# Merium88/3D-Object-Detection-of-Industrial-Joints

Measured on NVIDIA B200. Metric: SHOT descriptors/s + scene registrations/s at 1-8 B200 vs PCL OMP host CPU, higher is better.
Workload: dtype f32 (f64 for the SHOT frame/bin decisions)

## Files before the change

### 3d-object-detection-of-industrial-joints_b200/csrc/shot.cu

```cuda
#include <algorithm>

#include "linalg3.cuh"
#include "search.cuh"

namespace {

constexpr int SHOT_THREADS = 128;
constexpr int SHOT_LEN = 352;

__global__ void gather_normals_kernel(const float4 *__restrict__ sorted_pts, int n, const float4 *__restrict__ normals,
                                      float4 *__restrict__ out) {
  int i = blockIdx.x * blockDim.x + threadIdx.x;
  if (i < n) out[i] = normals[orig_index(sorted_pts[i])];
}

struct FloatBins {
  float *h;
  __device__ __forceinline__ void add(int bin, float v) const { atomicAdd(&h[bin], v); }
};
struct FixedBins {
  int *h;
  float scale;
  __device__ __forceinline__ void add(int bin, float v) const { atomicAdd(&h[bin], __float2int_rn(v * scale)); }
};

template <class Bins>
__device__ __noinline__ void shot_neighbor_exact(Bins s_hist, const float4 nv, const float4 p, const float4 c,
                                                 const float d2, const float *fr, const double radius) {
  const float fxx = fr[0], fxy = fr[1], fxz = fr[2];
  const float fyx = fr[3], fyy = fr[4], fyz = fr[5];
  const float fzx = fr[6], fzy = fr[7], fzz = fr[8];
  const double radius3_4 = (radius * 3) / 4, radius1_4 = radius / 4, radius1_2 = radius / 2;
  const double RAD_45 = 0.78539816339744830961566084581988;
  const double RAD_90 = 1.5707963267948966192313216916398;
  const double RAD_135 = 2.3561944901923449288469825374596;
  const double RAD_PI_7_8 = 2.7488935718910690836548129603691;
  {
        float dotf = nv.x * fzx;
        dotf += nv.y * fzy;
        dotf += nv.z * fzz;
        double cosineDesc = (double)dotf;
        if (cosineDesc > 1.0) cosineDesc = 1.0;
        if (cosineDesc < -1.0) cosineDesc = -1.0;
        double binDistance = ((1.0 + cosineDesc) * 10) / 2;
        const float dx = p.x - c.x, dy = p.y - c.y, dz = p.z - c.z;
        const double distance = sqrt((double)d2);
        if (fabs(distance) < 1E-15) return;
        float t;
        t = dx * fxx;
        t += dy * fxy;
        t += dz * fxz;
        double xInFeatRef = (double)t;
        t = dx * fyx;
        t += dy * fyy;
        t += dz * fyz;
        double yInFeatRef = (double)t;
        t = dx * fzx;
        t += dy * fzy;
        t += dz * fzz;
        double zInFeatRef = (double)t;
        if (fabs(yInFeatRef) < 1E-30) yInFeatRef = 0;
        if (fabs(xInFeatRef) < 1E-30) xInFeatRef = 0;
        if (fabs(zInFeatRef) < 1E-30) zInFeatRef = 0;

        const int bit4 = ((yInFeatRef > 0) || ((yInFeatRef == 0.0) && (xInFeatRef < 0))) ? 1 : 0;
        const int bit3 = (((xInFeatRef > 0) || ((xInFeatRef == 0.0) && (yInFeatRef > 0))) ? !bit4 : bit4) ? 1 : 0;
        int desc_index = (bit4 << 3) + (bit3 << 2);
        desc_index = desc_index << 1;
        if ((xInFeatRef * yInFeatRef > 0) || (xInFeatRef == 0.0))
          desc_index += (fabs(xInFeatRef) >= fabs(yInFeatRef)) ? 0 : 4;
        else
          desc_index += (fabs(xInFeatRef) > fabs(yInFeatRef)) ? 4 : 0;
        desc_index += zInFeatRef > 0 ? 1 : 0;
        desc_index += (distance > radius1_2) ? 2 : 0;

        const int step_index = (int)floor(binDistance + 0.5);
        const int volume_index = desc_index * 11;
        binDistance -= step_index;
        double intWeight = (1 - fabs(binDistance));
        if (binDistance > 0)
          s_hist.add(volume_index + ((step_index + 1) % 10), (float)binDistance);
        else
          s_hist.add(volume_index + ((step_index - 1 + 10) % 10), -(float)binDistance);
// ... 163 lines not shown
        if (pz) atomicAdd(&s_votes[2], pz);
      }
      __syncthreads();
      if (tid == 0) {
        double ax[2][3] = {{v1x, v1y, v1z}, {v3x, v3y, v3z}};
        for (int which = 0; which < 2; ++which) {
          int plus = 2 * s_votes[1 + which] - valid;
          double *a = ax[which];
          if (plus == 0) {
            const int med = valid / 2;
            for (int t = -2; t <= 2; ++t) {
              const float4 p = pts[pos[n_skip + med - t]];
              const double vx = (double)(p.x - c.x), vy = (double)(p.y - c.y), vz = (double)(p.z - c.z);
              if (vx * a[0] + vy * a[1] + vz * a[2] > 0) ++plus;
            }
            if (plus < 3) {
              a[0] = -a[0];
              a[1] = -a[1];
              a[2] = -a[2];
            }
          } else if (plus < 0) {
            a[0] = -a[0];
            a[1] = -a[1];
            a[2] = -a[2];
          }
        }
        const float x0 = (float)ax[0][0], x1 = (float)ax[0][1], x2 = (float)ax[0][2];
        const float z0 = (float)ax[1][0], z1 = (float)ax[1][1], z2 = (float)ax[1][2];
        s_frame[0] = x0;
        s_frame[1] = x1;
        s_frame[2] = x2;
        s_frame[3] = z1 * x2 - z2 * x1;
        s_frame[4] = z2 * x0 - z0 * x2;
        s_frame[5] = z0 * x1 - z1 * x0;
        s_frame[6] = z0;
        s_frame[7] = z1;
        s_frame[8] = z2;
      }
      __syncthreads();
    }

    if (lrf_only) {
      if (tid < 9) rf_out[(size_t)i * 9 + tid] = ok ? s_frame[tid] : nanf32();
      __syncthreads();
      continue;
    }

    const bool desc_ok = ok && n >= 5;
    if (desc_ok) {
      float fr[9];
#pragma unroll
      for (int a = 0; a < 9; ++a) fr[a] = s_frame[a];
      for (int j = tid; j < n; j += SHOT_THREADS) {
        const int pj = pos[j];
        const float4 nv = nrm[pj];
        if (!finite3(nv.x, nv.y, nv.z)) continue;
        shot_neighbor_exact(FloatBins{s_hist}, nv, pts[pj], c, key_d2(key[j]), fr, radius);
      }
      __syncthreads();
      double acc = 0.0;
      for (int b = tid; b < SHOT_LEN; b += SHOT_THREADS) {
        const float h = s_hist[b];
        acc += (double)(h * h);
      }
      acc = warp_sum(acc);
      if ((tid & 31) == 0) s_norm[tid >> 5] = acc;
      __syncthreads();
      const double acc_norm = sqrt(((s_norm[0] + s_norm[1]) + s_norm[2]) + s_norm[3]);
      const float fnorm = (float)acc_norm;
      for (int b = tid; b < SHOT_LEN; b += SHOT_THREADS) desc[(size_t)i * SHOT_LEN + b] = s_hist[b] / fnorm;
      if (rf_out && tid < 9) rf_out[(size_t)i * 9 + tid] = s_frame[tid];
    } else {
      for (int b = tid; b < SHOT_LEN; b += SHOT_THREADS) desc[(size_t)i * SHOT_LEN + b] = nanf32();
      if (rf_out && tid < 9) rf_out[(size_t)i * 9 + tid] = nanf32();
    }
    __syncthreads();
  }
}

constexpr int SW_WARPS = 8;
constexpr int SW_THREADS = SW_WARPS * 32;
constexpr int SW_CAP = 2016;

__global__ void __launch_bounds__(256)
    shot_count_cov_kernel(GridView g, const float4 *__restrict__ kp, int K, float radius_f, double radius, float r2,
                          int *__restrict__ counts, double *__restrict__ acc, unsigned long long *__restrict__ stats) {
  const int i = (blockIdx.x * blockDim.x + threadIdx.x) >> 5;
  const int lane = threadIdx.x & 31;
  if (i >= K) return;
  const float4 c = kp[i];
  double part[7] = {0, 0, 0, 0, 0, 0, 0};
  int n = 0, skipped = 0;
  int x0, x1, y0, y1, z0, z1;
  if (finite3(c.x, c.y, c.z) && g.n > 0 && ball_cell_range(g, c.x, c.y, c.z, radius_f, x0, x1, y0, y1, z0, z1)) {
    const float4 *__restrict__ pts = g.pts;
    const int *__restrict__ cs = g.cell_start;
    for (int z = z0; z <= z1; ++z)
      for (int y = y0; y <= y1; ++y) {
        const int base = g.dx * (y + g.dy * z);
        const int e = cs[base + x1 + 1];
        for (int j0 = cs[base + x0] + lane; j0 < e; j0 += 128) {
         float4 pp[4];
#pragma unroll
         for (int u = 0; u < 4; ++u) pp[u] = (j0 + 32 * u < e) ? pts[j0 + 32 * u] : make_float4(0.f, 0.f, 0.f, 0.f);
#pragma unroll
         for (int u = 0; u < 4; ++u) {
          const float4 p = pp[u];
          const float d2 = (j0 + 32 * u < e) ? sqdist3(c.x, c.y, c.z, p.x, p.y, p.z) : 3.0e38f;
          if (d2 < r2) {
            ++n;
            if (p.x == c.x && p.y == c.y && p.z == c.z) {
              ++skipped;
            } else {
              const double vx = (double)(p.x - c.x), vy = (double)(p.y - c.y), vz = (double)(p.z - c.z);
              const double w = radius - sqrt((double)d2);
              part[0] += w * (vx * vx);
              part[1] += w * (vx * vy);
              part[2] += w * (vx * vz);
              part[3] += w * (vy * vy);
              part[4] += w * (vy * vz);
              part[5] += w * (vz * vz);
              part[6] += w;
            }
          }
         }
        }
      }
  }
#pragma unroll
  for (int a = 0; a < 7; ++a) part[a] = warp_sum(part[a]);
  n = warp_sum(n);
  skipped = warp_sum(skipped);
  if (lane < 7) {
    double v = part[0];
#pragma unroll
    for (int a = 1; a < 7; ++a)
      if (lane == a) v = part[a];
    acc[(size_t)i * 8 + lane] = v;
  }
  if (lane == 7) acc[(size_t)i * 8 + 7] = (double)skipped;
  if (lane == 0) {
    counts[i] = n;
    if (stats) {
      atomicMax(&stats[0], (unsigned long long)n);
      atomicAdd(&stats[1], (unsigned long long)n);
    }
  }
}

__global__ void shot_eigen_kernel(const int *__restrict__ counts, const double *__restrict__ acc, int K,
                                  double *__restrict__ axes, int *__restrict__ flags) {
  const int i = blockIdx.x * blockDim.x + threadIdx.x;
  if (i >= K) return;
  const double *s = acc + (size_t)i * 8;
  const int valid = counts[i] - (int)s[7];
  int ok = valid >= 5 ? 1 : 0;
  double ax[6] = {0, 0, 0, 0, 0, 0};
  if (ok) {
    const double cov[9] = {s[0] / s[6], s[1] / s[6], s[2] / s[6], s[1] / s[6], s[3] / s[6],
                           s[4] / s[6], s[2] / s[6], s[4] / s[6], s[5] / s[6]};
    double w[3], V[9];
    eigh3_f64(cov, w, V);
    if (!isfinite(w[0]) || !isfinite(w[1]) || !isfinite(w[2])) ok = 0;
    ax[0] = V[0 * 3 + 2], ax[1] = V[1 * 3 + 2], ax[2] = V[2 * 3 + 2];
    ax[3] = V[0 * 3 + 0], ax[4] = V[1 * 3 + 0], ax[5] = V[2 * 3 + 0];
  }
#pragma unroll
  for (int a = 0; a < 6; ++a) axes[(size_t)i * 6 + a] = ax[a];
  flags[i] = ok;
}

struct ShotWarpSmem {
  int pos[SW_CAP];
  int hist[SHOT_LEN];
  int sel[8];
};

__global__ void __launch_bounds__(SW_THREADS, 3)
    shot_warp_kernel(GridView g, const float4 *__restrict__ nrm, const float4 *__restrict__ kp,
                     const int *__restrict__ counts, const double *__restrict__ acc, const double *__restrict__ axes,
                     const int *__restrict__ flags, int K, float radius_f, double radius, float r2,
                     int *__restrict__ work_counter, float *__restrict__ desc, float *__restrict__ rf_out,
                     int lrf_only) {
  extern __shared__ __align__(16) unsigned char smem_raw[];
  const int lane = threadIdx.x & 31, warp = threadIdx.x >> 5;
  ShotWarpSmem &sm = reinterpret_cast<ShotWarpSmem *>(smem_raw)[warp];
  const float4 *__restrict__ pts = g.pts;
  const int *__restrict__ cs = g.cell_start;

  const double radius3_4 = (radius * 3) / 4, radius1_4 = radius / 4, radius1_2 = radius / 2;
  const float r12f = (float)radius1_2, r34f = (float)radius3_4, r14f = (float)radius1_4;
  const float inv_r12f = 1.0f / r12f;
  const float m_r = 1e-6f * radius_f;
  const float RAD_45f = 0.78539816339744830961566084581988f, RAD_90f = 1.5707963267948966192313216916398f;
  const float RAD_135f = 2.3561944901923449288469825374596f, RAD_PI_7_8f = 2.7488935718910690836548129603691f;
  const float INV_RAD_90f = 1.0f / RAD_90f, INV_RAD_45f = 1.0f / RAD_45f;
  const float COS_45f = 0.70710678118654752440f;

  while (true) {
    int i = 0;
    if (lane == 0) i = atomicAdd(work_counter, 1);
    i = __shfl_sync(0xffffffffu, i, 0);
    if (i >= K) break;
    if (counts[i] > SW_CAP) continue;
    const float4 c = kp[i];

    int n = 0;
    {
      int x0, x1, y0, y1, z0, z1;
      if (finite3(c.x, c.y, c.z) && g.n > 0 && ball_cell_range(g, c.x, c.y, c.z, radius_f, x0, x1, y0, y1, z0, z1)) {
        for (int z = z0; z <= z1; ++z)
          for (int y = y0; y <= y1; ++y) {
            const int base = g.dx * (y + g.dy * z);
            const int s0 = cs[base + x0], e = cs[base + x1 + 1];
            for (int j0 = s0; j0 < e; j0 += 128) {
              float4 p[4];
#pragma unroll
              for (int u = 0; u < 4; ++u) {
                const int j = j0 + 32 * u + lane;
                p[u] = (j < e) ? pts[j] : make_float4(0.f, 0.f, 0.f, 0.f);
              }
#pragma unroll
              for (int u = 0; u < 4; ++u) {
                const int j = j0 + 32 * u + lane;
                const bool hit = j < e && sqdist3(c.x, c.y, c.z, p[u].x, p[u].y, p[u].z) < r2;
                const unsigned m = __ballot_sync(0xffffffffu, hit);
                if (hit) {
                  const int slot = n + __popc(m & ((1u << lane) - 1u));
                  if (slot < SW_CAP) sm.pos[slot] = j;
                }
                n += __popc(m);
              }
            }
          }
      }
    }
    if (n > SW_CAP) n = SW_CAP;
    for (int b = lane; b < SHOT_LEN; b += 32) sm.hist[b] = 0;
    __syncwarp();

    const int n_skip = (int)acc[(size_t)i * 8 + 7];
    const int valid = n - n_skip;
    const int ok = flags[i];
    double ax[6];
#pragma unroll
    for (int a = 0; a < 6; ++a) ax[a] = axes[(size_t)i * 6 + a];
    float fr[9];
    if (ok) {
      const float a0 = (float)ax[0], a1 = (float)ax[1], a2 = (float)ax[2];
      const float b0 = (float)ax[3], b1 = (float)ax[4], b2 = (float)ax[5];
      int px = 0, pz = 0;
      for (int j = lane; j < n; j += 32) {
        const float4 p = pts[sm.pos[j]];
        if (p.x == c.x && p.y == c.y && p.z == c.z) continue;
        const float fx = p.x - c.x, fy = p.y - c.y, fz = p.z - c.z;
        const float band = 4e-6f * (fabsf(fx) + fabsf(fy) + fabsf(fz));
        const float ex = fx * a0 + fy * a1 + fz * a2, ez = fx * b0 + fy * b1 + fz * b2;
        if (fabsf(ex) > band)
          px += ex > 0.f;
        else
          px += ((double)fx * ax[0] + (double)fy * ax[1] + (double)fz * ax[2] >= 0) ? 1 : 0;
        if (fabsf(ez) > band)
          pz += ez > 0.f;
        else
          pz += ((double)fx * ax[3] + (double)fy * ax[4] + (double)fz * ax[5] >= 0) ? 1 : 0;
      }
      px = warp_sum(px);
      pz = warp_sum(pz);
      const int plus_x = 2 * px - valid, plus_z = 2 * pz - valid;
      if (plus_x == 0 || plus_z == 0) {
        const int r0 = n_skip + valid / 2 - 2;
        const bool staged = n <= SW_CAP / 2;
        float *d2s = reinterpret_cast<float *>(sm.pos + SW_CAP / 2);
        auto d2_at = [&](int a) -> float {
          if (staged) return d2s[a];
          const float4 q = pts[sm.pos[a]];
          return sqdist3(c.x, c.y, c.z, q.x, q.y, q.z);
        };
        if (staged) {
          for (int a = lane; a < n; a += 32) {
            const float4 q = pts[sm.pos[a]];
            d2s[a] = sqdist3(c.x, c.y, c.z, q.x, q.y, q.z);
          }
          __syncwarp();
        }
        unsigned u_lo = 0, u_hi = 0;
#pragma unroll 1
        for (int which = 0; which < 2; ++which) {
          const int target = r0 + 4 * which + 1;
          unsigned lo = 0, hi = 0x7f800000u;
          while (lo < hi) {
// ... 145 lines not shown
            hist.add((desc_index - 2) * 11 + step_index, -rd);
          }
        } else {
          const float rd = (df - r14f) * inv_r12f;
          if (df < r14f)
            intWeight += 1 + rd;
          else {
            intWeight += 1 - rd;
            hist.add((desc_index + 2) * 11 + step_index, rd);
          }
        }
        const float inc = acosf(fminf(1.0f, fmaxf(-1.0f, cosv)));
        if (zf < 0.f) {
          const float id = (inc - RAD_135f) * INV_RAD_90f;
          if (cosv < -COS_45f)
            intWeight += 1 - id;
          else {
            intWeight += 1 + id;
            hist.add((desc_index + 1) * 11 + step_index, -id);
          }
        } else {
          const float id = (inc - RAD_45f) * INV_RAD_90f;
          if (cosv > COS_45f)
            intWeight += 1 + id;
          else {
            intWeight += 1 - id;
            hist.add((desc_index - 1) * 11 + step_index, id);
          }
        }
        {
          float ad = (az - az0) * INV_RAD_45f;
          ad = fmaxf(-0.5f, fminf(ad, 0.5f));
          if (ad > 0) {
            intWeight += 1 - ad;
            hist.add(((desc_index + 4) % 32) * 11 + step_index, ad);
          } else {
            intWeight += 1 + ad;
            hist.add(((desc_index - 4 + 32) % 32) * 11 + step_index, -ad);
          }
        }
        hist.add(volume_index + step_index, intWeight);
      }
      __syncwarp();
      double acc = 0.0;
      for (int b = lane; b < SHOT_LEN; b += 32) {
        const float h = (float)(unsigned)sm.hist[b] * fx_inv;
        acc += (double)(h * h);
      }
      acc = warp_sum(acc);
      const float fnorm = (float)sqrt(acc);
      for (int b = lane; b < SHOT_LEN; b += 32)
        desc[(size_t)i * SHOT_LEN + b] = ((float)(unsigned)sm.hist[b] * fx_inv) / fnorm;
      if (rf_out && lane < 9) {
        float v = 0.f;
#pragma unroll
        for (int a = 0; a < 9; ++a)
          if (lane == a) v = fr[a];
        rf_out[(size_t)i * 9 + lane] = v;
      }
    } else {
      for (int b = lane; b < SHOT_LEN; b += 32) desc[(size_t)i * SHOT_LEN + b] = nanf32();
      if (rf_out && lane < 9) rf_out[(size_t)i * 9 + lane] = nanf32();
    }
    __syncwarp();
  }
}

}

int dev_shot(b200_ctx *ctx, b200_cloud *c, const float *d_normals, const float4 *d_kp, int K, double radius,
             float *d_desc, float *d_rf, bool lrf_only) {
  if (!(radius > 0.0)) return ctx->fail(B200_ERR_INVALID, "shot: radius must be > 0");
  if (K <= 0) return B200_OK;
  const GridView *g;
  B200_TRY(cloud_grid_for_radius(c, radius, &g));
  DevBuf<int> counts, flags;
  DevBuf<double> acc, axes;
  DevBuf<unsigned long long> stats;
  B200_TRY(counts.alloc(ctx, (size_t)K));
  B200_TRY(flags.alloc(ctx, (size_t)K));
  B200_TRY(acc.alloc(ctx, (size_t)K * 8));
  B200_TRY(axes.alloc(ctx, (size_t)K * 6));
  B200_TRY(stats.alloc(ctx, 2));
  const float r2 = (float)(radius * radius);
  {
    StageScope stc_(ctx, ST_NBR_COUNT);
    B200_CUDA(ctx, cudaMemsetAsync(stats.p, 0, 2 * sizeof(unsigned long long), ctx->stream));
    shot_count_cov_kernel<<<ceil_div((long long)K * 32, 256), 256, 0, ctx->stream>>>(*g, d_kp, K, (float)radius, radius,
                                                                                    r2, counts.p, acc.p, stats.p);
    B200_LAUNCHED(ctx);
    shot_eigen_kernel<<<ceil_div(K, 128), 128, 0, ctx->stream>>>(counts.p, acc.p, K, axes.p, flags.p);
    B200_LAUNCHED(ctx);
  }
  unsigned long long hstats[2];
  B200_TRY(readback_small(ctx, stats.p, hstats, sizeof(hstats)));
  const int max_count = (int)hstats[0];
  ctx->last_max_nbrs = max_count;
  ctx->last_mean_nbrs = (double)hstats[1] / K;

  StageScope st_(ctx, ST_SHOT);
  DevBuf<float4> nrm_sorted;
  if (!lrf_only) {
    B200_TRY(nrm_sorted.alloc(ctx, (size_t)std::max(c->n_valid, 1)));
    if (c->n_valid > 0) {
      gather_normals_kernel<<<ceil_div(c->n_valid, 256), 256, 0, ctx->stream>>>(
          g->pts, c->n_valid, reinterpret_cast<const float4 *>(d_normals), nrm_sorted.p);
      B200_LAUNCHED(ctx);
    }
  }
  {
    DevBuf<int> work;
    B200_TRY(work.alloc(ctx, 1));
    B200_TRY(work.zero());
    const size_t smem_w = sizeof(ShotWarpSmem) * SW_WARPS;
    B200_CUDA(ctx, ensure_dyn_smem(shot_warp_kernel, smem_w));
    const int grid_w = std::min(ceil_div(K, SW_WARPS), ctx->sm_count * 3);
    shot_warp_kernel<<<grid_w, SW_THREADS, smem_w, ctx->stream>>>(*g, nrm_sorted.p, d_kp, counts.p, acc.p, axes.p, flags.p,
                                                                 K, (float)radius, radius, r2, work.p, d_desc, d_rf,
                                                                 lrf_only ? 1 : 0);
    B200_LAUNCHED(ctx);
  }
  if (max_count <= SW_CAP) return B200_OK;
  const int min_count = SW_CAP + 1;
  const int cap = next_pow2_host(std::max(max_count, 32));
  const size_t smem = (size_t)cap * 12;
  if (smem <= 96 * 1024) {
    B200_CUDA(ctx, ensure_dyn_smem(shot_kernel, smem));
    int per_sm = (int)std::max<size_t>(1, std::min<size_t>(8, (200 * 1024) / (smem + 4096)));
    const int grid = std::min(K, ctx->sm_count * per_sm);
    shot_kernel<<<grid, SHOT_THREADS, smem, ctx->stream>>>(*g, nrm_sorted.p, d_kp, K, (float)radius, radius, r2, cap,
                                                          nullptr, nullptr, d_desc, d_rf, lrf_only ? 1 : 0, counts.p, min_count);
    B200_LAUNCHED(ctx);
  } else {
    const int grid = std::min(K, ctx->sm_count * 2);
    DevBuf<unsigned long long> gk;
    DevBuf<int> gp;
    B200_TRY(gk.alloc(ctx, (size_t)grid * cap));
    B200_TRY(gp.alloc(ctx, (size_t)grid * cap));
    shot_kernel<<<grid, SHOT_THREADS, 0, ctx->stream>>>(*g, nrm_sorted.p, d_kp, K, (float)radius, radius, r2, cap,
                                                       gk.p, gp.p, d_desc, d_rf, lrf_only ? 1 : 0, counts.p, min_count);
    B200_LAUNCHED(ctx);
  }
  return B200_OK;
}
```

### 3d-object-detection-of-industrial-joints_b200/csrc/gc.cu

```cuda
#include <stdlib.h>
#include <string.h>

#include <algorithm>

#include "linalg3.cuh"
#include "pcl_eigen33.cuh"

namespace {

constexpr int RANK_ITEMS = 32;
constexpr int RANK_TILE = 2048;
__global__ void __launch_bounds__(256)
    gc_rank_kernel(const b200_corr *__restrict__ corrs, const int *__restrict__ d_C, int C_cap,
                   const float4 *__restrict__ model_kp, const float4 *__restrict__ scene_kp,
                   b200_corr *__restrict__ sorted, float4 *__restrict__ mp, float4 *__restrict__ sp,
                   const int *__restrict__ gate) {
  __shared__ unsigned long long tile[RANK_TILE];
  __shared__ int s_rank[RANK_ITEMS];
  if (gate && *gate == 0) return;
  const int C = min(*d_C, C_cap);
  if (blockIdx.x * RANK_ITEMS >= C) return;
  const int lane = threadIdx.x & 31, slice = threadIdx.x >> 5;
  const int i = blockIdx.x * RANK_ITEMS + lane;
  unsigned long long mykey = 0;
// ... 157 lines not shown
}

__device__ __forceinline__ int gc_row_words(int C) { return (((C + 31) >> 5) + 127) & ~127; }

__device__ __forceinline__ unsigned transpose32(unsigned x, int lane) {
#pragma unroll
  for (int s = 0; s < 5; ++s) {
    const int j = 16 >> s;
    const unsigned m = (s == 0) ? 0x0000ffffu : (s == 1) ? 0x00ff00ffu : (s == 2) ? 0x0f0f0f0fu : (s == 3) ? 0x33333333u : 0x55555555u;
    const unsigned y = __shfl_xor_sync(0xffffffffu, x, j);
    const bool upper = (lane & j) == 0;
    const unsigned a = upper ? x : y, b = upper ? y : x;
    const unsigned t = ((a >> j) ^ b) & m;
    x ^= upper ? (t << j) : t;
  }
  return x;
}

__global__ void __launch_bounds__(ADJ_THREADS)
    gc_adjacency_kernel(const float4 *__restrict__ mp, const float4 *__restrict__ sp, const int *__restrict__ d_C,
                        int C_cap, double gc_size, float g_lo, float g_hi, unsigned *__restrict__ adj) {
  __shared__ float4 s_m[ADJ_WORDS * 32];
  __shared__ float4 s_s[ADJ_WORDS * 32];
  __shared__ unsigned s_t[2][4][ADJ_ROWS];
  const int C = min(*d_C, C_cap);
  const int row_words = gc_row_words(C);
  const int w0 = blockIdx.x * ADJ_WORDS;
  const int i0 = blockIdx.y * ADJ_ROWS;
  if (w0 >= row_words || i0 >= C) return;
  if ((w0 + ADJ_WORDS) * 32 <= i0) return;
  const int tid = threadIdx.x;
  for (int t = tid; t < ADJ_WORDS * 32; t += ADJ_THREADS) {
    const int j = w0 * 32 + t;
    const bool in = j < C;
    s_m[t] = in ? mp[j] : make_float4(0.f, 0.f, 0.f, 0.f);
    s_s[t] = in ? sp[j] : make_float4(0.f, 0.f, 0.f, 0.f);
  }
  __syncthreads();
  const int lane = tid & 31;
  const int i = i0 + (tid & (ADJ_ROWS - 1));
  const int half = tid / ADJ_ROWS, wr = (tid & (ADJ_ROWS - 1)) >> 5;
  const int wbase = (tid / ADJ_ROWS) * (ADJ_WORDS / 2);
  const bool valid = i < C;
  const float4 mi = valid ? mp[i] : make_float4(0.f, 0.f, 0.f, 0.f);
  const float4 si = valid ? sp[i] : make_float4(0.f, 0.f, 0.f, 0.f);
  unsigned *row = adj + (size_t)(valid ? i : 0) * row_words + w0 + wbase;
#pragma unroll 1
  for (int wq = 0; wq < ADJ_WORDS / 2; wq += 4) {
    const int gw0 = w0 + wbase + wq;
    if (gw0 >= row_words) break;
    const int jg = gw0 * 32;
    if (jg + 128 <= i0) continue;
    const bool mirror = jg >= i0 + ADJ_ROWS;
    unsigned out[4];
#pragma unroll
    for (int w4 = 0; w4 < 4; ++w4) {
      const int w = wq + w4;
      unsigned bits = 0;
      const int t0 = (wbase + w) * 32;
#pragma unroll ADJ_UNROLL_N
      for (int b = 0; b < 32; ++b) {
        const bool ok = gc_fits(mi, si, s_m[t0 + b], s_s[t0 + b], g_lo, g_hi, gc_size);
        bits |= (ok ? 1u : 0u) << b;
      }
      const int gw = gw0 + w4;
      const int j0 = gw * 32;
      if (j0 + 32 > C) bits &= (j0 >= C) ? 0u : ((1u << (C - j0)) - 1u);
      if ((i >> 5) == gw) bits &= ~(1u << (i & 31));
      if (!valid) bits = 0u;
      out[w4] = bits;
      if (mirror)
        s_t[half][wr][w4 * 32 + lane] = transpose32(bits, lane);
    }
    if (mirror) {
      asm volatile("bar.sync %0, %1;" ::"r"(1 + half), "r"(ADJ_ROWS) : "memory");
      const int col = tid & (ADJ_ROWS - 1);
      if (jg + col < C)
        *reinterpret_cast<uint4 *>(adj + (size_t)(jg + col) * row_words + (i0 >> 5)) =
            make_uint4(s_t[half][0][col], s_t[half][1][col], s_t[half][2][col], s_t[half][3][col]);
      asm volatile("bar.sync %0, %1;" ::"r"(1 + half), "r"(ADJ_ROWS) : "memory");
    }
    if (valid) *reinterpret_cast<uint4 *>(row + wq) = make_uint4(out[0], out[1], out[2], out[3]);
  }
}

constexpr int GW = 16;
constexpr int GG_THREADS = GW * 32;
constexpr int G_MC = 64;
constexpr int G_HS = 4096;
constexpr int G_LIST = 64;

struct GroupArgs {
  const unsigned *adj;
  const float4 *mp;
  const float4 *sp;
  int *overflow;
  int *members;
  int *inst_offsets;
  int *n_inst_out;
  long long *dbg;
};

__device__ __forceinline__ int warp_incl_scan(int v, int lane) {
#pragma unroll
  for (int o = 1; o < 32; o <<= 1) {
    const int t = __shfl_up_sync(0xffffffffu, v, o);
    if (lane >= o) v += t;
  }
  return v;
}

__device__ __forceinline__ unsigned gc_hash(int m) { return ((unsigned)m * 2654435761u) >> 20; }

__device__ __forceinline__ int first_bit128(const uint4 &w, int base) {
  if (w.x) return base + __ffs(w.x) - 1;
  if (w.y) return base + 32 + __ffs(w.y) - 1;
  if (w.z) return base + 64 + __ffs(w.z) - 1;
  if (w.w) return base + 96 + __ffs(w.w) - 1;
  return 0x7fffffff;
}

__global__ void __launch_bounds__(GG_THREADS, 1)
    gc_group_kernel(GroupArgs ga, const int *__restrict__ d_C, int C_cap, int dyn_smem_bytes, double gc_size, float g_lo,
                    float g_hi, int gc_threshold, int max_inst, const int *__restrict__ gate) {
  extern __shared__ __align__(16) unsigned char s_raw[];
  if (gate && *gate == 0) return;
  __shared__ int s_seed[GW], s_size[GW], s_conf[GW];
  __shared__ int s_nwin, s_big;
  __shared__ int s_hkey[G_HS], s_hval[G_HS];
  __shared__ int s_mem[GW][G_MC];
  __shared__ int s_list[GW][64];
  __shared__ float4 s_newm[GW], s_news[GW];
  const int tid = threadIdx.x, lane = tid & 31, warp = tid >> 5;
  const int C = min(*d_C, C_cap);
  const int row_words = gc_row_words(C);
  const int nq = row_words >> 7;
  const int gw = min(GW, dyn_smem_bytes / (row_words * 4) - 1);
  uint4 *s_taken4 = reinterpret_cast<uint4 *>(s_raw);
  unsigned *s_taken = reinterpret_cast<unsigned *>(s_raw);
  uint4 *my_cb4 = s_taken4 + (size_t)(row_words >> 2) * (1 + warp);

  for (int w = tid; w < row_words; w += GG_THREADS) {
    const int j0 = w * 32;
    s_taken[w] = (j0 + 32 <= C) ? 0u : ((j0 >= C) ? ~0u : ~((1u << (C - j0)) - 1u));
  }
  for (int h = tid; h < G_HS; h += GG_THREADS) {
    s_hkey[h] = -1;
    s_hval[h] = 0x7fffffff;
  }
  if (tid == 0) ga.inst_offsets[0] = 0;
  int cur = 0, n_inst = 0, total = 0;
  __syncthreads();

  int *my_mem = s_mem[warp];
  int *my_over = ga.overflow + (size_t)warp * C_cap;

#ifdef B200_GC_TIMING
  long long t_win = 0, t_eval = 0, t_commit = 0, n_rounds = 0, t_wait = 0;
#define GC_CLOCK(v) const long long v = clock64()
#define GC_ACC(acc, expr) acc += (expr)
#else
#define GC_CLOCK(v)
#define GC_ACC(acc, expr)
#endif
  while (true) {
    GC_CLOCK(c0);
// ... 1578 lines not shown
      if (t < n) f = ((double)residual2(s_bestT, rb.mp[mem[t]], rb.sp[mem[t]]) < thresh2) ? 1 : 0;
      const unsigned m = __ballot_sync(0xffffffffu, f);
      if (lane == 0) s_warp_cnt[warp] = __popc(m);
      __syncthreads();
      int before = n_inl, chunk_total = 0;
      for (int w = 0; w < RS_THREADS / 32; ++w) {
        if (w < warp) before += s_warp_cnt[w];
        chunk_total += s_warp_cnt[w];
      }
      if (f) flags[before + __popc(m & ((1u << lane) - 1u))] = t;
      n_inl += chunk_total;
      __syncthreads();
    }
  }
  __syncthreads();
  const bool use_model = ok && n_inl >= 3;
  float *T = rb.T_out + (size_t)b * 16;
  if (tid < 16) T[tid] = use_model ? s_bestT[tid] : ((tid % 5 == 0) ? 1.0f : 0.0f);
  const int out_n = use_model ? n_inl : n;
  for (int i = tid; i < out_n; i += RS_THREADS) {
    const int t = use_model ? last_pos[flags[i]] : i;
    if (off + i < corr_cap) rb.inst_corrs[off + i] = rb.sorted[mem[t]];
  }
  if (tid == 0) rb.inst_counts[b] = out_n;
}

}

int dev_gc(b200_ctx *ctx, const float4 *d_model_kp, const float4 *d_scene_kp, const b200_corr *d_corrs,
           const int *d_C, int C_cap, double gc_size, int gc_threshold, float *d_T, int max_inst, int *d_inst_offsets,
           int *d_inst_counts, b200_corr *d_inst_corrs, int corr_cap, int *d_n_inst) {
  if (max_inst < 1) return ctx->fail(B200_ERR_INVALID, "gc: max_inst must be >= 1");
  B200_CUDA(ctx, cudaMemsetAsync(d_n_inst, 0, sizeof(int), ctx->stream));
  B200_CUDA(ctx, cudaMemsetAsync(d_inst_offsets, 0, sizeof(int) * ((size_t)max_inst + 1), ctx->stream));
  B200_CUDA(ctx, cudaMemsetAsync(d_inst_counts, 0, sizeof(int) * (size_t)max_inst, ctx->stream));
  if (C_cap <= 0) return B200_OK;
  constexpr int GC_ASYNC_CAP = 32768;
  constexpr long long GC_MAX_C = 524288;
  int C_eff = C_cap;
  if (C_cap > GC_ASYNC_CAP) {
    int C_now = 0;
    B200_TRY(readback_small(ctx, d_C, &C_now, sizeof(int)));
    C_eff = std::max(1, std::min(C_now, C_cap));
    if (C_eff > GC_MAX_C) return ctx->fail(B200_ERR_CAPACITY, "gc: more than 524288 correspondences");
  }
  const int row_words_cap = ((((C_eff + 31) >> 5) + 127) & ~127);
  const float g_lo = nextafterf((float)gc_size, -INFINITY), g_hi = nextafterf((float)gc_size, INFINITY);
  DevBuf<b200_corr> sorted;
  DevBuf<float4> mp, sp;
  DevBuf<unsigned> adj;
  DevBuf<int> overflow, members, fb, sort_fb;
  B200_TRY(sorted.alloc(ctx, (size_t)C_eff));
  B200_TRY(sort_fb.alloc(ctx, 1));
  B200_TRY(mp.alloc(ctx, (size_t)C_eff));
  B200_TRY(sp.alloc(ctx, (size_t)C_eff));
  B200_TRY(adj.alloc(ctx, (size_t)C_eff * row_words_cap));
  {
    StageScope st_(ctx, ST_GC_SORT);
    const char *sel = getenv("B200_GC_SORT");
    const int *gate = nullptr;
    if (!(sel && !strcmp(sel, "count"))) {
      DevBuf<int> hist, start;
      DevBuf<unsigned long long> keys;
      B200_TRY(hist.alloc(ctx, SORT_BUCKETS));
      B200_TRY(start.alloc(ctx, SORT_BUCKETS + 1));
      B200_TRY(keys.alloc(ctx, (size_t)C_eff));
      B200_TRY(hist.zero());
      const int nblk = ceil_div(C_eff, 256);
      gc_sort_hist_kernel<<<nblk, 256, 0, ctx->stream>>>(d_corrs, d_C, C_eff, hist.p);
      B200_LAUNCHED(ctx);
      gc_sort_scan_kernel<<<1, 1024, 0, ctx->stream>>>(hist.p, start.p, sort_fb.p);
      B200_LAUNCHED(ctx);
      gc_sort_scatter_kernel<<<nblk, 256, 0, ctx->stream>>>(d_corrs, d_C, C_eff, start.p, hist.p, keys.p, sort_fb.p);
      B200_LAUNCHED(ctx);
      gc_sort_rank_kernel<<<nblk, 256, 0, ctx->stream>>>(d_corrs, d_C, C_eff, d_model_kp, d_scene_kp, start.p, keys.p,
                                                        sorted.p, mp.p, sp.p, sort_fb.p);
      B200_LAUNCHED(ctx);
      gate = sort_fb.p;
    }
    gc_rank_kernel<<<ceil_div(C_eff, RANK_ITEMS), 256, 0, ctx->stream>>>(d_corrs, d_C, C_eff, d_model_kp, d_scene_kp,
                                                                 sorted.p, mp.p, sp.p, gate);
    B200_LAUNCHED(ctx);
  }
  {
    StageScope st_(ctx, ST_GC_ADJ);
    dim3 grid(ceil_div(row_words_cap, ADJ_WORDS), ceil_div(C_eff, ADJ_ROWS));
    gc_adjacency_kernel<<<grid, ADJ_THREADS, 0, ctx->stream>>>(mp.p, sp.p, d_C, C_eff, gc_size, g_lo, g_hi, adj.p);
    B200_LAUNCHED(ctx);
  }
  B200_TRY(overflow.alloc(ctx, (size_t)std::max(GW, GCL) * C_eff));
  B200_TRY(members.alloc(ctx, (size_t)C_eff));
  B200_TRY(fb.alloc(ctx, 16));
  GroupArgs ga;
  ga.adj = adj.p;
  ga.mp = mp.p;
  ga.sp = sp.p;
  ga.overflow = overflow.p;
  ga.members = members.p;
  ga.inst_offsets = d_inst_offsets;
  ga.n_inst_out = d_n_inst;
  DevBuf<long long> dbg;
  const bool debug = getenv("B200_GC_DEBUG") != nullptr;
  ga.dbg = nullptr;
  if (debug) {
    B200_TRY(dbg.alloc(ctx, 256));
    B200_TRY(dbg.zero());
    ga.dbg = dbg.p;
  }
  if (ctx->wide) ctx->wide->leave();
  {
    StageScope st_(ctx, ST_GC_GROUP);
    const size_t row_bytes = (size_t)row_words_cap * sizeof(unsigned);
    const char *sel = getenv("B200_GC_GROUP");
    const bool use_stream = sel && !strcmp(sel, "stream") && row_words_cap <= GS_MAX_ROW_WORDS;
    const int *gate = nullptr;
    if (use_stream) {
      B200_CUDA(ctx, cudaMemsetAsync(fb.p, 0, 16 * sizeof(int), ctx->stream));
      const size_t smem = (size_t)GS_MAX_ROW_WORDS * 4 + (size_t)GS_NBLK * GS_BLK;
      B200_CUDA(ctx, ensure_dyn_smem(gc_group_stream_kernel, smem));
      gc_group_stream_kernel<<<1, GS_THREADS, smem, ctx->stream>>>(ga, d_C, C_eff, gc_size, g_lo, g_hi, gc_threshold, max_inst,
                                                                  fb.p);
      B200_LAUNCHED(ctx);
      gate = fb.p;
    }
    const bool use_cluster = !(sel && !strcmp(sel, "cta")) && 2 * row_bytes <= 200 * 1024;
    if (use_cluster) {
      const size_t smem = 2 * row_bytes;
      B200_CUDA(ctx, ensure_dyn_smem(gc_group_cluster_kernel, smem));
      gc_group_cluster_kernel<<<GCL, GCL_THREADS, smem, ctx->stream>>>(ga, d_C, C_eff, gc_size, g_lo, g_hi, gc_threshold,
                                                                      max_inst, gate);
      B200_LAUNCHED(ctx);
    } else {
      const size_t budget = 160 * 1024;
      if (2 * row_bytes > budget) return ctx->fail(B200_ERR_CAPACITY, "gc: too many correspondences for the grouping kernel");
      const size_t smem = std::min(budget, row_bytes * (size_t)(1 + GW));
      B200_CUDA(ctx, ensure_dyn_smem(gc_group_kernel, smem));
      gc_group_kernel<<<1, GG_THREADS, smem, ctx->stream>>>(ga, d_C, C_eff, (int)smem, gc_size, g_lo, g_hi, gc_threshold,
                                                            max_inst, gate);
      B200_LAUNCHED(ctx);
    }
  }
  if (debug) {
    int f[16];
    B200_CUDA(ctx, cudaMemcpyAsync(f, fb.p, sizeof(f), cudaMemcpyDeviceToHost, ctx->stream));
    B200_CUDA(ctx, ctx->sync());
    fprintf(stderr, "gc_group stream: handed over %d, wait %d ticket %d | issue %d take %d head %d tail %d end %d\n", f[0], f[1], f[2],
            f[3], f[4], f[5], f[6], f[7]);
  }
  if (debug && getenv("B200_GC_STREAM_TIMING")) {
    long long h[256];
    B200_CUDA(ctx, cudaMemcpyAsync(h, dbg.p, sizeof(h), cudaMemcpyDeviceToHost, ctx->stream));
    B200_CUDA(ctx, ctx->sync());
    for (int w = 0; w < 1 + GS_PROD + GS_CONS; ++w)
      fprintf(stderr,
              w == 0 ? "dispatcher %2d: wait-free %lld pick %lld (%lld %lld %lld %lld %lld) tickets %lld\n"
                     : (w <= GS_PROD ? "producer %2d: wait-turn %lld row %lld wait-ring %lld list %lld gather %lld (%lld %lld) slots %lld\n"
                                     : "consumer %2d: wait-ready %lld grow %lld wait-commit %lld commit %lld [validate %lld in-turn %lld] regrown %lld slots %lld\n"),
              w, h[w * 8], h[w * 8 + 1], h[w * 8 + 2], h[w * 8 + 3], h[w * 8 + 4], h[w * 8 + 5], h[w * 8 + 6], h[w * 8 + 7]);
  } else if (debug) {
    long long h[GW * 8];
    B200_CUDA(ctx, cudaMemcpyAsync(h, dbg.p, sizeof(h), cudaMemcpyDeviceToHost, ctx->stream));
    B200_CUDA(ctx, ctx->sync());
    for (int w = 0; w < GCL; ++w)
      fprintf(stderr, "gc_group cta %d: window %lld init %lld and %lld list %lld list+greedy %lld cluster-sync %lld commit %lld rounds %lld\n",
              w, h[w * 8], h[w * 8 + 1], h[w * 8 + 2], h[w * 8 + 3], h[w * 8 + 4], h[w * 8 + 5], h[w * 8 + 6], h[w * 8 + 7]);
  }

  return dev_ransac_instances(ctx, sorted.p, mp.p, sp.p, members.p, d_inst_offsets, d_n_inst, C_eff, gc_size, d_T, max_inst,
                              d_inst_counts, d_inst_corrs, corr_cap);
}

int dev_ransac_instances(b200_ctx *ctx, const b200_corr *d_corrs, const float4 *d_mp, const float4 *d_sp,
                         const int *d_members, const int *d_inst_offsets, const int *d_n_inst, int C_cap,
                         double threshold, float *d_T, int max_inst, int *d_inst_counts, b200_corr *d_inst_corrs,
                         int corr_cap) {
  DevBuf<int> shuffled, last_pos, flags;
  if (!ctx->mt_state) {
    unsigned host_state[624];
    mt19937_twisted_state(12345u, host_state);
    B200_CUDA(ctx, cudaMalloc(&ctx->mt_state, sizeof(host_state)));
    B200_CUDA(ctx, cudaMemcpyAsync(ctx->mt_state, host_state, sizeof(host_state), cudaMemcpyHostToDevice, ctx->stream));
    B200_CUDA(ctx, ctx->sync());
  }
  B200_TRY(shuffled.alloc(ctx, (size_t)C_cap));
  B200_TRY(last_pos.alloc(ctx, (size_t)C_cap));
// ... 23 lines not shown
```

Measured before the change: 23.98 million.

## Record neighbor indices in count pass and reuse them in SHOT warp kernel

The count/covariance kernel now uses warp ballots to compact in-radius neighbor indices into a per-keypoint global list, capped by a budget (default 1024). The SHOT warp kernel loads that list into shared memory instead of rescanning grid cells when the count fits the budget. This removes the second radius search at the cost of extra global writes and reads (up to K*budget ints of memory) and more work inside the count kernel. An environment variable can restore the old scan path.

Result: faster. 24.57 million (median of 6 runs) (+2.5%).

```diff
diff --git a/3d-object-detection-of-industrial-joints_b200/csrc/shot.cu b/3d-object-detection-of-industrial-joints_b200/csrc/shot.cu
--- a/3d-object-detection-of-industrial-joints_b200/csrc/shot.cu
+++ b/3d-object-detection-of-industrial-joints_b200/csrc/shot.cu
@@ -1,4 +1,6 @@
 #include <algorithm>
+#include <cstdlib>
+#include <cstring>
 
 #include "linalg3.cuh"
 #include "search.cuh"
@@ -328,12 +330,15 @@
 constexpr int SW_THREADS = SW_WARPS * 32;
 constexpr int SW_CAP = 2016;
 
-__global__ void __launch_bounds__(256)
+template <bool kList>
+__global__ void __launch_bounds__(256, 4)
     shot_count_cov_kernel(GridView g, const float4 *__restrict__ kp, int K, float radius_f, double radius, float r2,
-                          int *__restrict__ counts, double *__restrict__ acc, unsigned long long *__restrict__ stats) {
+                          int *__restrict__ counts, double *__restrict__ acc, unsigned long long *__restrict__ stats,
+                          int *__restrict__ list_pos, int budget) {
   const int i = (blockIdx.x * blockDim.x + threadIdx.x) >> 5;
   const int lane = threadIdx.x & 31;
   if (i >= K) return;
+  int *__restrict__ list = kList ? list_pos + (size_t)i * budget : nullptr;
   const float4 c = kp[i];
   double part[7] = {0, 0, 0, 0, 0, 0, 0};
   int n = 0, skipped = 0;
@@ -345,16 +350,25 @@
       for (int y = y0; y <= y1; ++y) {
         const int base = g.dx * (y + g.dy * z);
         const int e = cs[base + x1 + 1];
-        for (int j0 = cs[base + x0] + lane; j0 < e; j0 += 128) {
+        for (int j0 = cs[base + x0]; j0 < e; j0 += 128) {
          float4 pp[4];
 #pragma unroll
-         for (int u = 0; u < 4; ++u) pp[u] = (j0 + 32 * u < e) ? pts[j0 + 32 * u] : make_float4(0.f, 0.f, 0.f, 0.f);
+         for (int u = 0; u < 4; ++u) {
+          const int j = j0 + 32 * u + lane;
+          pp[u] = (j < e) ? pts[j] : make_float4(0.f, 0.f, 0.f, 0.f);
+         }
 #pragma unroll
          for (int u = 0; u < 4; ++u) {
           const float4 p = pp[u];
-          const float d2 = (j0 + 32 * u < e) ? sqdist3(c.x, c.y, c.z, p.x, p.y, p.z) : 3.0e38f;
+          const int j = j0 + 32 * u + lane;
+          const float d2 = (j < e) ? sqdist3(c.x, c.y, c.z, p.x, p.y, p.z) : 3.0e38f;
+          const unsigned m = __ballot_sync(0xffffffffu, d2 < r2);
+          if (kList && d2 < r2) {
+            const int slot = n + __popc(m & ((1u << lane) - 1u));
+            if (slot < budget) list[slot] = j;
+          }
+          n += __popc(m);
           if (d2 < r2) {
-            ++n;
             if (p.x == c.x && p.y == c.y && p.z == c.z) {
               ++skipped;
             } else {
@@ -375,7 +389,6 @@
   }
 #pragma unroll
   for (int a = 0; a < 7; ++a) part[a] = warp_sum(part[a]);
-  n = warp_sum(n);
   skipped = warp_sum(skipped);
   if (lane < 7) {
     double v = part[0];
@@ -425,9 +438,9 @@
 __global__ void __launch_bounds__(SW_THREADS, 3)
     shot_warp_kernel(GridView g, const float4 *__restrict__ nrm, const float4 *__restrict__ kp,
                      const int *__restrict__ counts, const double *__restrict__ acc, const double *__restrict__ axes,
-                     const int *__restrict__ flags, int K, float radius_f, double radius, float r2,
-                     int *__restrict__ work_counter, float *__restrict__ desc, float *__restrict__ rf_out,
-                     int lrf_only) {
+                     const int *__restrict__ flags, const int *__restrict__ list_pos, int budget,
+                     int K, float radius_f, double radius, float r2, int *__restrict__ work_counter,
+                     float *__restrict__ desc, float *__restrict__ rf_out, int lrf_only) {
   extern __shared__ __align__(16) unsigned char smem_raw[];
   const int lane = threadIdx.x & 31, warp = threadIdx.x >> 5;
   ShotWarpSmem &sm = reinterpret_cast<ShotWarpSmem *>(smem_raw)[warp];
@@ -448,11 +461,16 @@
     if (lane == 0) i = atomicAdd(work_counter, 1);
     i = __shfl_sync(0xffffffffu, i, 0);
     if (i >= K) break;
-    if (counts[i] > SW_CAP) continue;
+    const int count = counts[i];
+    if (count > SW_CAP) continue;
     const float4 c = kp[i];
 
     int n = 0;
-    {
+    if (list_pos && count <= budget) {
+      n = count;
+      const int *__restrict__ list = list_pos + (size_t)i * budget;
+      for (int a = lane; a < n; a += 32) sm.pos[a] = list[a];
+    } else {
       int x0, x1, y0, y1, z0, z1;
       if (finite3(c.x, c.y, c.z) && g.n > 0 && ball_cell_range(g, c.x, c.y, c.z, radius_f, x0, x1, y0, y1, z0, z1)) {
         for (int z = z0; z <= z1; ++z)
@@ -764,12 +782,27 @@
   B200_TRY(acc.alloc(ctx, (size_t)K * 8));
   B200_TRY(axes.alloc(ctx, (size_t)K * 6));
   B200_TRY(stats.alloc(ctx, 2));
+  const char *sel = getenv("B200_SHOT_LIST");
+  const bool use_list = !(sel && !strcmp(sel, "scan"));
+  int budget = 0;
+  DevBuf<int> list_pos;
+  if (use_list) {
+    const char *bs = getenv("B200_SHOT_LIST_BUDGET");
+    budget = (int)std::min(std::max(bs ? atoll(bs) : 1024LL, 0LL), (long long)SW_CAP);
+    budget = (int)std::min<long long>(budget, (1LL << 28) / K);
+    B200_TRY(list_pos.alloc(ctx, std::max<size_t>((size_t)K * budget, 1)));
+  }
   const float r2 = (float)(radius * radius);
   {
     StageScope stc_(ctx, ST_NBR_COUNT);
     B200_CUDA(ctx, cudaMemsetAsync(stats.p, 0, 2 * sizeof(unsigned long long), ctx->stream));
-    shot_count_cov_kernel<<<ceil_div((long long)K * 32, 256), 256, 0, ctx->stream>>>(*g, d_kp, K, (float)radius, radius,
-                                                                                    r2, counts.p, acc.p, stats.p);
+    const int grid_c = ceil_div((long long)K * 32, 256);
+    if (use_list)
+      shot_count_cov_kernel<true><<<grid_c, 256, 0, ctx->stream>>>(*g, d_kp, K, (float)radius, radius, r2, counts.p,
+                                                                   acc.p, stats.p, list_pos.p, budget);
+    else
+      shot_count_cov_kernel<false><<<grid_c, 256, 0, ctx->stream>>>(*g, d_kp, K, (float)radius, radius, r2, counts.p,
+                                                                    acc.p, stats.p, nullptr, 0);
     B200_LAUNCHED(ctx);
     shot_eigen_kernel<<<ceil_div(K, 128), 128, 0, ctx->stream>>>(counts.p, acc.p, K, axes.p, flags.p);
     B200_LAUNCHED(ctx);
@@ -798,8 +831,8 @@
     B200_CUDA(ctx, ensure_dyn_smem(shot_warp_kernel, smem_w));
     const int grid_w = std::min(ceil_div(K, SW_WARPS), ctx->sm_count * 3);
     shot_warp_kernel<<<grid_w, SW_THREADS, smem_w, ctx->stream>>>(*g, nrm_sorted.p, d_kp, counts.p, acc.p, axes.p, flags.p,
-                                                                 K, (float)radius, radius, r2, work.p, d_desc, d_rf,
-                                                                 lrf_only ? 1 : 0);
+                                                                 use_list ? list_pos.p : nullptr, budget, K, (float)radius, radius, r2, work.p,
+                                                                 d_desc, d_rf, lrf_only ? 1 : 0);
     B200_LAUNCHED(ctx);
   }
   if (max_count <= SW_CAP) return B200_OK;
```

## Add register-blocked geometric-consistency adjacency kernel with fast-path and exact fallback

Applied to the files above, without the earlier changes.

Replaces the default adjacency bitmap kernel with a register-blocked version in which each thread handles R=4 rows and a warp sweeps R words, reusing shared-memory tiles of model/scene points. It computes a fast approximate consistency bit per pair and tracks how close each word comes to the threshold boundary. Only ambiguous words are recomputed through the exact gc_fits path. Mirrored columns are written through a register transpose instead of shared-memory barriers. The cost is a tolerance bound whose correctness depends on the error analysis, more register pressure, and env-selectable variants plus a bitmap dump for debugging.

Result: no change. 23.95 million before, 23.78 million after, median of 6 (-0.7%).

```diff
diff --git a/3d-object-detection-of-industrial-joints_b200/csrc/gc.cu b/3d-object-detection-of-industrial-joints_b200/csrc/gc.cu
--- a/3d-object-detection-of-industrial-joints_b200/csrc/gc.cu
+++ b/3d-object-detection-of-industrial-joints_b200/csrc/gc.cu
@@ -263,6 +263,153 @@
     }
     if (valid) *reinterpret_cast<uint4 *>(row + wq) = make_uint4(out[0], out[1], out[2], out[3]);
   }
+}
+
+#ifndef ADJ_RB_UNROLL
+#define ADJ_RB_UNROLL 8
+#endif
+constexpr int ADJ_RB_UNROLL_N = ADJ_RB_UNROLL;
+
+__device__ __forceinline__ float dist2f_fused(const float4 &a, const float4 &b) {
+  const float d0 = a.x - b.x, d1 = a.y - b.y, d2 = a.z - b.z;
+  return __fmaf_rn(d2, d2, __fmaf_rn(d1, d1, d0 * d0));
+}
+
+__device__ __forceinline__ float norm3f(const float4 &p) { return sqrtf(p.x * p.x + p.y * p.y + p.z * p.z); }
+
+__device__ __forceinline__ float fmin_nan(float a, float b) {
+  float r;
+  asm("min.NaN.f32 %0, %1, %2;" : "=f"(r) : "f"(a), "f"(b));
+  return r;
+}
+
+__device__ __forceinline__ float fmax_nan(float a, float b) {
+  float r;
+  asm("max.NaN.f32 %0, %1, %2;" : "=f"(r) : "f"(a), "f"(b));
+  return r;
+}
+
+__device__ __noinline__ unsigned gc_word_exact(float4 mi, float4 si, const float4 *cm, const float4 *cs, float g_lo,
+                                               float g_hi, double gc_size, unsigned long long *n_exact) {
+  unsigned bits = 0;
+  int n = 0;
+  for (int b = 0; b < 32; ++b) {
+    bits |= (gc_fits(mi, si, cm[b], cs[b], g_lo, g_hi, gc_size) ? 1u : 0u) << b;
+    if (n_exact) {
+      const float sa = sqrt_approx(dist2f(si, cs[b])), sc = sqrt_approx(dist2f(mi, cm[b]));
+      const float diff = fabsf(sa - sc), tol = 1e-6f * (sa + sc) + 1e-15f;
+      n += (!(diff > g_hi + tol) && !(diff < g_lo - tol)) ? 1 : 0;
+    }
+  }
+  if (n_exact) {
+    atomicAdd(n_exact, 1ull);
+    atomicAdd(n_exact + 1, (unsigned long long)n);
+  }
+  return bits;
+}
+
+template <int R_, int MINB>
+__global__ void __launch_bounds__(256, MINB)
+    gc_adjacency_rb_kernel(const float4 *__restrict__ mp, const float4 *__restrict__ sp, const int *__restrict__ d_C,
+                           int C_cap, double gc_size, float g_lo, float g_hi, unsigned *__restrict__ adj,
+                           unsigned long long *__restrict__ n_exact) {
+  constexpr int R = R_, ROWS = 32 * R, WORDS = 8 * R;
+  __shared__ float4 s_m[WORDS * 32];
+  __shared__ float4 s_s[WORDS * 32];
+  __shared__ int s_nmax;
+  const int C = min(*d_C, C_cap);
+  const int row_words = gc_row_words(C);
+  const int w0 = blockIdx.x * WORDS;
+  const int i0 = blockIdx.y * ROWS;
+  if (w0 >= row_words || i0 >= C) return;
+  if ((w0 + WORDS) * 32 <= i0) return;
+  const int tid = threadIdx.x, lane = tid & 31, warp = tid >> 5;
+  if (tid == 0) s_nmax = 0;
+  __syncthreads();
+  float nmax = 0.f;
+  for (int t = tid; t < WORDS * 32; t += 256) {
+    const int j = w0 * 32 + t;
+    float4 m = make_float4(0.f, 0.f, 0.f, 0.f), s = m;
+    if (j < C) {
+      m = mp[j];
+      s = sp[j];
+      nmax = fmax_nan(nmax, norm3f(m) + norm3f(s));
+    }
+    s_m[t] = m;
+    s_s[t] = s;
+  }
+  atomicMax(&s_nmax, nmax != nmax ? 0x7fffffff : __float_as_int(nmax));
+  __syncthreads();
+  const int gw0 = w0 + warp * R;
+  const int jg = gw0 * 32;
+  if (jg < i0) return;
+  const bool mirror = jg > i0;
+  const float g = (float)gc_size;
+  const float tile_n = __int_as_float(s_nmax);
+  float4 mi[R], si[R];
+  float thr[R];
+  bool valid[R];
+#pragma unroll
+  for (int k = 0; k < R; ++k) {
+    const int i = i0 + 32 * k + lane;
+    valid[k] = i < C;
+    mi[k] = valid[k] ? mp[i] : make_float4(0.f, 0.f, 0.f, 0.f);
+    si[k] = valid[k] ? sp[i] : make_float4(0.f, 0.f, 0.f, 0.f);
+    thr[k] = 1.001e-6f * (norm3f(mi[k]) + norm3f(si[k]) + tile_n) + 1e-15f + 2.f * (g_hi - g_lo);
+  }
+  unsigned out[R][R];
+#pragma unroll 1
+  for (int w = 0; w < R; ++w) {
+    const int gw = gw0 + w, j0 = gw * 32;
+    unsigned bits[R];
+#pragma unroll
+    for (int k = 0; k < R; ++k) bits[k] = 0u;
+    if (j0 < C) {
+      const float4 *cm = s_m + (warp * R + w) * 32, *cs = s_s + (warp * R + w) * 32;
+      float amb[R];
+#pragma unroll
+      for (int k = 0; k < R; ++k) amb[k] = __int_as_float(0x7f800000);
+#pragma unroll ADJ_RB_UNROLL_N
+      for (int b = 31; b >= 0; --b) {
+        const float4 mj = cm[b], sj = cs[b];
+#pragma unroll
+        for (int k = 0; k < R; ++k) {
+          const float y = fabsf(sqrt_approx(dist2f_fused(si[k], sj)) - sqrt_approx(dist2f_fused(mi[k], mj))) - g;
+          amb[k] = fmin_nan(amb[k], fabsf(y));
+          bits[k] = (bits[k] << 1) | (__float_as_uint(y) >> 31);
+        }
+      }
+#pragma unroll
+      for (int k = 0; k < R; ++k) {
+        if (valid[k] && !(amb[k] > thr[k])) bits[k] = gc_word_exact(mi[k], si[k], cm, cs, g_lo, g_hi, gc_size, n_exact);
+        if (j0 + 32 > C) bits[k] &= (1u << (C - j0)) - 1u;
+        const int i = i0 + 32 * k + lane;
+        if ((i >> 5) == gw) bits[k] &= ~(1u << (i & 31));
+        if (!valid[k]) bits[k] = 0u;
+      }
+      if (mirror) {
+        unsigned col[R];
+#pragma unroll
+        for (int k = 0; k < R; ++k) col[k] = transpose32(bits[k], lane);
+        if (j0 + lane < C) {
+          if constexpr (R == 4) *reinterpret_cast<uint4 *>(adj + (size_t)(j0 + lane) * row_words + (i0 >> 5)) = make_uint4(col[0], col[1], col[2], col[3]);
+          else *reinterpret_cast<uint2 *>(adj + (size_t)(j0 + lane) * row_words + (i0 >> 5)) = make_uint2(col[0], col[R - 1]);
+        }
+      }
+    }
+#pragma unroll
+    for (int k = 0; k < R; ++k) {
+#pragma unroll
+      for (int q = 0; q + 1 < R; ++q) out[k][q] = out[k][q + 1];
+      out[k][R - 1] = bits[k];
+    }
+  }
+#pragma unroll
+  for (int k = 0; k < R; ++k)
+    if (valid[k]) {
+      if constexpr (R == 4) *reinterpret_cast<uint4 *>(adj + (size_t)(i0 + 32 * k + lane) * row_words + gw0) = make_uint4(out[k][0], out[k][1], out[k][2], out[k][3]);
+      else *reinterpret_cast<uint2 *>(adj + (size_t)(i0 + 32 * k + lane) * row_words + gw0) = make_uint2(out[k][0], out[k][R - 1]);
+    }
 }
 
 constexpr int GW = 16;
@@ -2007,11 +2154,54 @@
                                                                  sorted.p, mp.p, sp.p, gate);
     B200_LAUNCHED(ctx);
   }
+  const bool debug = getenv("B200_GC_DEBUG") != nullptr;
   {
     StageScope st_(ctx, ST_GC_ADJ);
-    dim3 grid(ceil_div(row_words_cap, ADJ_WORDS), ceil_div(C_eff, ADJ_ROWS));
-    gc_adjacency_kernel<<<grid, ADJ_THREADS, 0, ctx->stream>>>(mp.p, sp.p, d_C, C_eff, gc_size, g_lo, g_hi, adj.p);
-    B200_LAUNCHED(ctx);
+    const char *sel = getenv("B200_GC_ADJ");
+    if (sel && !strcmp(sel, "classic")) {
+      dim3 grid(ceil_div(row_words_cap, ADJ_WORDS), ceil_div(C_eff, ADJ_ROWS));
+      gc_adjacency_kernel<<<grid, ADJ_THREADS, 0, ctx->stream>>>(mp.p, sp.p, d_C, C_eff, gc_size, g_lo, g_hi, adj.p);
+      B200_LAUNCHED(ctx);
+    } else {
+      DevBuf<unsigned long long> n_exact;
+      if (debug) {
+        B200_TRY(n_exact.alloc(ctx, 2));
+        B200_TRY(n_exact.zero());
+      }
+      if (sel && !strcmp(sel, "r2")) {
+        dim3 grid(ceil_div(row_words_cap, 16), ceil_div(C_eff, 64));
+        gc_adjacency_rb_kernel<2, 0><<<grid, 256, 0, ctx->stream>>>(mp.p, sp.p, d_C, C_eff, gc_size, g_lo, g_hi, adj.p, n_exact.p);
+      } else if (sel && !strcmp(sel, "r4m3")) {
+        dim3 grid(ceil_div(row_words_cap, 32), ceil_div(C_eff, 128));
+        gc_adjacency_rb_kernel<4, 3><<<grid, 256, 0, ctx->stream>>>(mp.p, sp.p, d_C, C_eff, gc_size, g_lo, g_hi, adj.p, n_exact.p);
+      } else {
+        dim3 grid(ceil_div(row_words_cap, 32), ceil_div(C_eff, 128));
+        gc_adjacency_rb_kernel<4, 0><<<grid, 256, 0, ctx->stream>>>(mp.p, sp.p, d_C, C_eff, gc_size, g_lo, g_hi, adj.p, n_exact.p);
+      }
+      B200_LAUNCHED(ctx);
+      if (debug) {
+        unsigned long long h[2];
+        B200_CUDA(ctx, cudaMemcpyAsync(h, n_exact.p, sizeof(h), cudaMemcpyDeviceToHost, ctx->stream));
+        B200_CUDA(ctx, ctx->sync());
+        fprintf(stderr, "gc_adjacency: C %d, %llu row words re-tested, %llu pairs to the exact expression\n", C_eff, h[0], h[1]);
+      }
+    }
+  }
+  if (const char *path = getenv("B200_GC_ADJ_DUMP")) {
+    int C_now = 0;
+    B200_TRY(readback_small(ctx, d_C, &C_now, sizeof(int)));
+    C_now = std::min(C_now, C_eff);
+    const size_t words = (size_t)C_now * (((((C_now + 31) >> 5) + 127) & ~127));
+    unsigned *h = (unsigned *)malloc(std::max<size_t>(words, 1) * sizeof(unsigned));
+    if (!h) return ctx->fail(B200_ERR_NOMEM, "gc: bitmap dump: out of host memory");
+    cudaError_t e = cudaMemcpyAsync(h, adj.p, words * sizeof(unsigned), cudaMemcpyDeviceToHost, ctx->stream);
+    if (e == cudaSuccess) e = cudaStreamSynchronize(ctx->stream);
+    FILE *f = e == cudaSuccess ? fopen(path, "wb") : nullptr;
+    const bool ok = f && fwrite(h, sizeof(unsigned), words, f) == words;
+    if (f) fclose(f);
+    free(h);
+    B200_CUDA(ctx, e);
+    if (!ok) return ctx->fail(B200_ERR_INVALID, "gc: bitmap dump: cannot write the file");
   }
   B200_TRY(overflow.alloc(ctx, (size_t)std::max(GW, GCL) * C_eff));
   B200_TRY(members.alloc(ctx, (size_t)C_eff));
@@ -2025,7 +2215,6 @@
   ga.inst_offsets = d_inst_offsets;
   ga.n_inst_out = d_n_inst;
   DevBuf<long long> dbg;
-  const bool debug = getenv("B200_GC_DEBUG") != nullptr;
   ga.dbg = nullptr;
   if (debug) {
     B200_TRY(dbg.alloc(ctx, 256));
```
